# danielreardon/scintools

Hardware: NVIDIA H100
Metric: theta-theta eta-trials/sec on 4096x8192 dynspec (higher is better)
Workload: dtype f32

## Files before the change

profiles/probe_build_gather.py:

```python
import argparse
import ctypes
import json
import os
import subprocess
import sys

ROOT = os.path.dirname(os.path.dirname(os.path.abspath(__file__)))
sys.path.insert(0, ROOT)
import numpy as np
import torch

import bench as B
from scintools_b200 import _device as D, _lib, ththmod as thth


def load(path):
    lib = ctypes.CDLL(os.path.abspath(path))
    for name in ("sb_init", "sb_last_error", "sb_profile_enable", "sb_profile_collect",
                 "sb_eta_sweep", "sb_cs_f32", "sb_cs_bound_f32", "sb_release"):
        fn, ref = getattr(lib, name), getattr(_lib.lib, name)
        fn.restype, fn.argtypes = ref.restype, ref.argtypes
    if lib.sb_init(torch.cuda.current_device()) != 0:
        raise RuntimeError(lib.sb_last_error().decode())
    return lib


def check(lib, rc):
    if rc != 0:
        raise RuntimeError("error %d: %s" % (rc, lib.sb_last_error().decode()))


def stats(v):
    v = np.asarray(v, float)
    return {"min": float(v.min()), "median": float(np.median(v)), "max": float(v.max())}


def main():
    ap = argparse.ArgumentParser()
    ap.add_argument("libs", nargs="+", help="name=path, the first one is the reference")
    ap.add_argument("--rounds", type=int, default=10)
    ap.add_argument("--steps", type=int, default=20)
    ap.add_argument("--warmup", type=int, default=3)
    ap.add_argument("--out", default=None)
    a = ap.parse_args()
    card = subprocess.run(["nvidia-smi", "--query-gpu=name,power.limit,clocks.max.sm",
                           "--format=csv,noheader"], capture_output=True, text=True).stdout.strip()
    print("card:", card)
    D.device()
    libs = [(s.split("=", 1)[0], load(s.split("=", 1)[1])) for s in a.libs]

    dyn, freq, t = B.make_dynspec()
    fd = np.asarray(thth.fft_axis(t, "mHz", B.NPAD))
    tau = np.asarray(thth.fft_axis(freq, "us", B.NPAD))
    edges = np.linspace(-B.EDGE_LIM, B.EDGE_LIM, B.NEDGE)
    rng = np.random.default_rng(11)
    lim_nu = B.EDGE_LIM * (1.0 - 1.0 / (B.NEDGE - 1))
    edges_nu = np.sort(rng.uniform(-lim_nu, lim_nu, B.NEDGE))
    d_dyn = D.upload(dyn)
    ntau, nfd = (B.NPAD + 1) * B.NF, (B.NPAD + 1) * B.NT
    pitch = nfd // 2 + 16
    d_cs = D.empty((ntau, pitch, 2), torch.float32)
    keep = thth.needed_fd_columns(fd, edges) or 0
    d_bound = D.empty((1,), torch.float32)
    cs = thth.DeviceCS(d_cs, nfd=nfd, ncols_valid=keep or None, bound=d_bound)
    stream = D.stream_ptr()

    def buffers(etas):
        n = len(etas)
        return dict(n=n, etas=D.upload(np.ascontiguousarray(etas)),
                    eigs=D.empty((n,), torch.float64), stat=D.empty((n,), torch.int32),
                    nred=D.empty((n,), torch.int32), iters=D.empty((n,), torch.int32))

    def sweep(lib, geom, buf):
        check(lib, lib.sb_eta_sweep(geom.ref, buf["etas"].data_ptr(), buf["n"], thth.DEFAULT_TOL, 0,
                                    buf["eigs"].data_ptr(), buf["stat"].data_ptr(),
                                    buf["nred"].data_ptr(), buf["iters"].data_ptr(), stream))

    def spectrum(lib):
        check(lib, lib.sb_cs_f32(d_dyn.data_ptr(), B.NF, B.NT, B.NPAD, 0.0, 0, 1, pitch, keep,
                                 d_cs.data_ptr(), stream))
        check(lib, lib.sb_cs_bound_f32(d_dyn.data_ptr(), B.NF, B.NT, B.NPAD, 0.0,
                                       d_bound.data_ptr(), stream))

    def timed(lib, step, steps):
        lib.sb_profile_enable(1)
        e0, e1 = torch.cuda.Event(enable_timing=True), torch.cuda.Event(enable_timing=True)
        torch.cuda.synchronize()
        e0.record()
        for _ in range(steps):
            step()
        e1.record()
        torch.cuda.synchronize()
        ms = np.zeros(16)
        cnt = np.zeros(16, dtype=np.int32)
        check(lib, lib.sb_profile_collect(ms.ctypes.data, cnt.ctypes.data, 16))
        lib.sb_profile_enable(0)
        kern = {n_: ms[i] / steps for i, n_ in enumerate(B.PROF_NAMES) if cnt[i]}
        return e0.elapsed_time(e1) / steps, kern

    def ab(label, geom, etas, with_cs, rounds, steps):
        buf = buffers(etas)
        res = {name: {"step_ms": [], "kernel_ms": {}} for name, _ in libs}
        outs = {}
        for name, lib in libs:
            def step(lib=lib):
                if with_cs:
                    spectrum(lib)
                sweep(lib, geom, buf)
            for _ in range(a.warmup):
                step()
            torch.cuda.synchronize()
            outs[name] = {k: buf[k].cpu().numpy().copy() for k in ("eigs", "stat", "nred", "iters")}
            res[name]["step"] = step
        for _ in range(rounds):
            for name, lib in libs:
                ms, kern = timed(lib, res[name]["step"], steps)
                res[name]["step_ms"].append(ms)
                for k, v in kern.items():
                    res[name]["kernel_ms"].setdefault(k, []).append(v)
        ref = outs[libs[0][0]]
        out = {}
        for name, _ in libs:
            o = outs[name]
            same = all(np.array_equal(o[k], ref[k], equal_nan=(k == "eigs")) for k in o)
            out[name] = {"step_ms": stats(res[name]["step_ms"]),
                         "kernel_ms": {k: stats(v) for k, v in res[name]["kernel_ms"].items()},
                         "bit_equal_to_" + libs[0][0]: bool(same)}
            print(label, name, json.dumps(out[name]))
        return out

    geom = thth._Geom(cs, tau, fd, edges, True)
    geom_nu = thth._Geom(cs, tau, fd, edges_nu, True)
    report = {"card": card, "rounds": a.rounds, "steps": a.steps}
    report["bench_step_1024_uniform"] = ab("bench_step_1024_uniform", geom, B.eta_grid(B.NETA), True,
                                           a.rounds, a.steps)
    spectrum(libs[0][1])
    torch.cuda.synchronize()
    short = max(3, a.rounds // 2)
    report["sweep_16_uniform"] = ab("sweep_16_uniform", geom, B.eta_grid(16), False, short, a.steps)
    report["sweep_1024_nonuniform"] = ab("sweep_1024_nonuniform", geom_nu, B.eta_grid(B.NETA), False,
                                         short, max(2, a.steps // 4))
    report["sweep_16_nonuniform"] = ab("sweep_16_nonuniform", geom_nu, B.eta_grid(16), False, short,
                                       a.steps)
    for _, lib in libs:
        lib.sb_release()
    line = json.dumps(report)
    print(line)
    if a.out:
        os.makedirs(os.path.dirname(os.path.abspath(a.out)), exist_ok=True)
        with open(a.out, "w") as fh:
            fh.write(line + "\n")


if __name__ == "__main__":
    main()
```

scintools_b200/csrc/eig_half.cu:

```cuda
#ifndef SB_HOST_EMU
#include <cuda_fp16.h>
#endif
#include <float.h>
#include <math.h>
#include <stdlib.h>

#include "lanczos.cuh"
#include "tma.cuh"

namespace sb {

enum { EB_ST_INDEX_ERROR = 1, EB_ST_ZERO_START = 2, EB_ST_TOO_SMALL = 4,
       EB_ST_NOT_CONVERGED = 8 };

constexpr int EB_THREADS = 256;
constexpr int EB_NW = EB_THREADS / 32;
constexpr int EB_NST = 2;
#ifdef SB_EB_SLOTS
constexpr int EB_SLOTS = SB_EB_SLOTS;
#else
constexpr int EB_SLOTS = 48;
#endif

__device__ __forceinline__ void ffma2(float2& acc, const float2 a, const float b) {
    acc.x = fmaf(a.x, b, acc.x);
    acc.y = fmaf(a.y, b, acc.y);
}

__device__ __forceinline__ float2 unpack_f16x2(const unsigned p) {
    __half2 h;
    *reinterpret_cast<unsigned*>(&h) = p;
    return __half22float2(h);
}

__device__ __forceinline__ unsigned pack_h2(const float lo, const float hi) {
#ifdef SB_HOST_EMU
    const __half2 h = __floats2half2_rn(lo, hi);
    return (unsigned)h.x | ((unsigned)h.y << 16);
#else
    unsigned r;
    asm("cvt.rn.f16x2.f32 %0, %1, %2;" : "=r"(r) : "f"(hi), "f"(lo));
    return r;
#endif
}

constexpr int EB_TC_NST = 5;
#define EB_OWN5(a, b, c, d, e, cnt) \
    ((unsigned)(a) | (unsigned)(b) << 5 | (unsigned)(c) << 10 | (unsigned)(d) << 15 | \
     (unsigned)(e) << 20 | (unsigned)(cnt) << 25)
__device__ __forceinline__ unsigned eb_own_pack(const int warp) {
    if (warp >= EB_NW) return 0u;
    return EB_OWN5(warp, 15 - warp, 16 + warp, 31 - warp, 0, 4);
}

#ifdef SB_HOST_EMU
inline void ldsm_x4(unsigned (&r)[4], smem_addr a) {
    unsigned long long all[32];
    emu::warp_gather((unsigned long long)(uintptr_t)a, all);
    const int lane = (int)(threadIdx.x & 31), g = lane >> 2, t = lane & 3;
    for (int i = 0; i < 4; ++i)
        std::memcpy(&r[i], (const unsigned char*)(uintptr_t)all[8 * i + g] + 4 * t, 4);
}
inline void ldsm_x4_t(unsigned (&r)[4], smem_addr a) {
    unsigned long long all[32];
    emu::warp_gather((unsigned long long)(uintptr_t)a, all);
    const int lane = (int)(threadIdx.x & 31), g = lane >> 2, t = lane & 3;
    for (int i = 0; i < 4; ++i) {
        unsigned short lo, hi;
        std::memcpy(&lo, (const unsigned char*)(uintptr_t)all[8 * i + 2 * t] + 2 * g, 2);
        std::memcpy(&hi, (const unsigned char*)(uintptr_t)all[8 * i + 2 * t + 1] + 2 * g, 2);
        r[i] = (unsigned)lo | ((unsigned)hi << 16);
    }
}
inline void mma16816(float (&d)[4], const unsigned (&a)[4], const unsigned b0, const unsigned b1) {
    unsigned long long A01[32], A23[32], Bq[32];
    emu::warp_gather((unsigned long long)a[0] | ((unsigned long long)a[1] << 32), A01);
    emu::warp_gather((unsigned long long)a[2] | ((unsigned long long)a[3] << 32), A23);
    emu::warp_gather((unsigned long long)b0 | ((unsigned long long)b1 << 32), Bq);
    const int lane = (int)(threadIdx.x & 31), g = lane >> 2, t = lane & 3;
    auto half_of = [](unsigned w, int hi) { return emu_h2f((unsigned short)(hi ? w >> 16 : w & 0xffffu)); };
    auto Aat = [&](int row, int k) {
        const int ln = (row & 7) * 4 + ((k & 7) >> 1);
        const unsigned long long w = (k < 8) ? A01[ln] : A23[ln];
        return half_of((unsigned)(row < 8 ? w : w >> 32), k & 1);
    };
    auto Bat = [&](int k, int n) {
        const unsigned long long w = Bq[n * 4 + ((k & 7) >> 1)];
        return half_of((unsigned)(k < 8 ? w : w >> 32), k & 1);
    };
    for (int q = 0; q < 4; ++q) {
        const int row = g + 8 * (q >> 1), col = 2 * t + (q & 1);
        float acc = d[q];
        for (int k = 0; k < 16; ++k) acc += Aat(row, k) * Bat(k, col);
        d[q] = acc;
    }
}
#else
__device__ __forceinline__ void ldsm_x4(unsigned (&r)[4], const smem_addr a) {
    asm volatile("ldmatrix.sync.aligned.m8n8.x4.shared.b16 {%0, %1, %2, %3}, [%4];"
                 : "=r"(r[0]), "=r"(r[1]), "=r"(r[2]), "=r"(r[3]) : "r"(a) : "memory");
}
__device__ __forceinline__ void ldsm_x4_t(unsigned (&r)[4], const smem_addr a) {
    asm volatile("ldmatrix.sync.aligned.m8n8.x4.trans.shared.b16 {%0, %1, %2, %3}, [%4];"
                 : "=r"(r[0]), "=r"(r[1]), "=r"(r[2]), "=r"(r[3]) : "r"(a) : "memory");
}
__device__ __forceinline__ void mma16816(float (&d)[4], const unsigned (&a)[4], const unsigned b0,
                                         const unsigned b1) {
    asm("mma.sync.aligned.m16n8k16.row.col.f32.f16.f16.f32 {%0, %1, %2, %3}, {%4, %5, %6, %7}, "
        "{%8, %9}, {%0, %1, %2, %3};"
        : "+f"(d[0]), "+f"(d[1]), "+f"(d[2]), "+f"(d[3])
        : "r"(a[0]), "r"(a[1]), "r"(a[2]), "r"(a[3]), "r"(b0), "r"(b1));
}
#endif

__host__ __device__ constexpr size_t eig_half_slice() {
    return (size_t)EB_TC_NST * 1024 + 4096;
}
__host__ __device__ inline size_t eig_half_smem(int ld) {
    return sizeof(LanczosShared) + 4 * (size_t)ld * sizeof(float2) +
           (size_t)EB_NW * eig_half_slice() + (size_t)EB_NW * EB_NST * 8 + 16 +
           4 * (size_t)(ld / 2) * 8;
}

__global__ void __launch_bounds__(EB_THREADS + 32, 2)
thth_eig_half_kernel(const float2* __restrict__ Mbase, const unsigned* __restrict__ Mbbase,
                     int ld, const int* __restrict__ nred, int eta0,
                     double* __restrict__ eigs, int* __restrict__ status,
                     int* __restrict__ iters, double tol, double etol, double etol_h, double rtol_r,
                     int max_iter, float2* __restrict__ gbasis) {
    extern __shared__ __align__(128) unsigned char smem_raw[];
    LanczosShared& S = *reinterpret_cast<LanczosShared*>(smem_raw);
    float2* v = reinterpret_cast<float2*>(smem_raw + sizeof(LanczosShared));
    float2* vp = v + ld;
    float2* w = vp + ld;
    float2* u = w + ld;
    unsigned char* ring = reinterpret_cast<unsigned char*>(u + ld);
    float2* part = reinterpret_cast<float2*>(ring);
    constexpr int WSL = (int)eig_half_slice();
    static_assert(WSL >= EB_NST * 4096, "the fp32 pass needs two 4 KB stages per warp");
    unsigned long long* mbar = reinterpret_cast<unsigned long long*>(ring + (size_t)EB_NW * WSL);
    uint2* P = reinterpret_cast<uint2*>(reinterpret_cast<unsigned char*>(mbar) +
                                        (size_t)EB_NW * EB_NST * 8 + 16);
    const int tid = threadIdx.x, lane = tid & 31;
    const int warp = __shfl_sync(0xffffffffu, tid >> 5, 0);
    constexpr int CHKW = EB_NW;
    const bool worker = warp < EB_NW;
    const int tidw = worker ? tid : (1 << 24);
    const int e = blockIdx.x;
    const int n = nred[eta0 + e];
    const float2* M = Mbase + (size_t)e * ld * ld;
    const unsigned* Mb = Mbbase + (size_t)e * ld * ld;
    float2* basis = gbasis + (size_t)e * EB_SLOTS * ld;
    const double qnan = __longlong_as_double(0x7ff8000000000000LL);

    if (status[eta0 + e] & EB_ST_INDEX_ERROR) {
        if (tid == 0) { eigs[eta0 + e] = qnan; iters[eta0 + e] = 0; }
        return;
    }
    if (n < 3) {
        if (tid == 0) {
            eigs[eta0 + e] = qnan; iters[eta0 + e] = 0;
            status[eta0 + e] |= EB_ST_TOO_SMALL;
        }
        return;
    }
    for (int i = tidw; i < EB_NW * WSL / 16; i += EB_THREADS)
        reinterpret_cast<float4*>(ring)[i] = make_float4(0.f, 0.f, 0.f, 0.f);
    if (tid == 0) {
        for (int i = 0; i < EB_NW * EB_NST; ++i) mbar_init(mbar + i, 1);
        fence_mbarrier_init();
    }
    fence_proxy_async();
    __syncthreads();
    const int ncol4 = (n + 1) >> 1;
    unsigned char* mystage = ring + (size_t)warp * WSL;
    unsigned long long* mybar = mbar + EB_NST * warp;
    unsigned phbits = 0;

    auto matvec_t = [&](int check_m, double et) {
        const int ldh = ld >> 1;
        for (int c = tidw; c < ld; c += EB_THREADS) w[c] = make_float2(0.f, 0.f);
        for (int i = tidw; i < ldh; i += EB_THREADS) {
            const float4 x = *reinterpret_cast<const float4*>(v + 2 * i);
            const unsigned xr = pack_h2(x.x, x.z), xi = pack_h2(x.y, x.w);
            const float2 hr = unpack_f16x2(xr), hi = unpack_f16x2(xi);
            const unsigned lr = pack_h2((x.x - hr.x) * 2048.f, (x.z - hr.y) * 2048.f);
            const unsigned li = pack_h2((x.y - hi.x) * 2048.f, (x.w - hi.y) * 2048.f);
            const int q = (((i >> 3) << 2) + (i & 3)) * 2 + ((i >> 2) & 1);
            P[q] = make_uint2(xr, xi ^ 0x80008000u);
            P[ldh + q] = make_uint2(xi, xr);
            P[2 * ldh + q] = make_uint2(lr, li ^ 0x80008000u);
            P[3 * ldh + q] = make_uint2(li, lr);
        }
        unsigned char* wring = ring + (size_t)warp * WSL;
        float4* mypart = reinterpret_cast<float4*>(wring + EB_TC_NST * 1024);
        if (worker) {
#pragma unroll
            for (int i = 0; i < 8; ++i) mypart[lane + 32 * i] = make_float4(0.f, 0.f, 0.f, 0.f);
        }
        __syncthreads();
        const int g = lane >> 2, t = lane & 3;
        const int NI = (n + 14) >> 4;
        const int NH = (n + 15) >> 4;
        const int NGL = ld >> 3;
        const unsigned own = eb_own_pack(warp);
        const int cnt = (int)(own >> 25);
        const smem_addr sbase = smem_addr_of(wring);
        smem_addr cdst = sbase + lane * 16;
        const unsigned char* gsrc = reinterpret_cast<const unsigned char*>(Mb) + lane * 16;
        const int mi = lane >> 3;
        const int arow = (lane & 7) + 8 * (mi & 1), trow = (lane & 7) + 8 * (mi >> 1);
        smem_addr aoff = sbase + arow * 32 + ((((mi >> 1) & 1) ^ ((arow >> 2) & 1)) << 4);
        smem_addr toff = sbase + trow * 32 + (((mi & 1) ^ ((trow >> 2) & 1)) << 4);
#ifndef SB_HOST_EMU
        asm volatile("" : "+r"(cdst), "+r"(aoff), "+r"(toff), "+l"(gsrc));
#endif
        constexpr unsigned RING_BYTES = EB_TC_NST * 1024;
        int pj = -1, prem = 0;
        unsigned pa = 0u, pst = 0u;
        unsigned cst = 0u;
        bool pend = false;
        auto fetch_next = [&]() {
            if (prem == 0 && !pend) {
                for (;;) {
                    if (++pj >= cnt) { pend = true; break; }
                    const int I = (int)((own >> (5 * pj)) & 31u);
                    if (I < NI) {
                        prem = NH - I;
                        pa = (unsigned)(I * NGL + 2 * I) << 9;
                        break;
                    }
                }
            }
            if (!pend) {
                cp_async16_s(cdst + pst, gsrc + pa);
                cp_async16_s(cdst + pst + 512u, gsrc + pa + 512u);
                pa += 1024u;
                --prem;
            }
            pst += 1024u;
            if (pst == RING_BYTES) pst = 0u;
            cp_async_commit();
        };
        for (int k = 0; k < EB_TC_NST - 1; ++k) fetch_next();
        if (check_m > 0 && warp == CHKW) lanczos_check(S, check_m, tol, et);
        const float lo_scale = 1.f / 2048.f;
        const bool bact = g < 4;
        const uint4* Pg = reinterpret_cast<const uint4*>(P + (g & 3) * ldh) + t;
        for (int j = 0; j < cnt; ++j) {
            const int I = (int)((own >> (5 * j)) & 31u);
            if (I >= NI) continue;
            const uint4* pb = Pg + 4 * I;
            unsigned tb0 = 0u, tb1 = 0u;
            if (bact) { const uint4 e4 = *pb; tb0 = e4.x; tb1 = e4.z; }
            float acc[4] = {0.f, 0.f, 0.f, 0.f};
            float4* pc = mypart + 8 * I + g;
            for (int h = I; h < NH; ++h) {
                uint4 bq = make_uint4(0u, 0u, 0u, 0u);
                if (bact) bq = *pb;
                float4 q = make_float4(0.f, 0.f, 0.f, 0.f);
                if (t == 0) q = *pc;
                cp_async_wait<EB_TC_NST - 2>();
                __syncwarp();
                unsigned a0[4], t0[4], a1[4], t1[4];
                ldsm_x4(a0, aoff + cst);
                ldsm_x4_t(t0, toff + cst);
                ldsm_x4(a1, aoff + cst + 512u);
                ldsm_x4_t(t1, toff + cst + 512u);
                fetch_next();
                float c0[4] = {0.f, 0.f, 0.f, 0.f}, c1[4] = {0.f, 0.f, 0.f, 0.f};
                mma16816(acc, a0, bq.x, bq.y);
                mma16816(c0, t0, tb0, tb1);
                mma16816(acc, a1, bq.z, bq.w);
                mma16816(c1, t1, tb0, tb1);
                cst += 1024u;
                if (cst == RING_BYTES) cst = 0u;
                const float yr0 = c0[0] + c0[3], yi0 = c0[1] - c0[2];
                const float yr1 = c1[0] + c1[3], yi1 = c1[1] - c1[2];
                const float lr0 = __shfl_xor_sync(0xffffffffu, yr0, 1), li0 = __shfl_xor_sync(0xffffffffu, yi0, 1);
                const float lr1 = __shfl_xor_sync(0xffffffffu, yr1, 1), li1 = __shfl_xor_sync(0xffffffffu, yi1, 1);
                if (t == 0) {
                    q.x += fmaf(lr0, lo_scale, yr0);
                    q.y += fmaf(li0, lo_scale, yi0);
                    q.z += fmaf(lr1, lo_scale, yr1);
                    q.w += fmaf(li1, lo_scale, yi1);
                    *pc = q;
                }
                pb += 4;
                pc += 8;
            }
            const float l0 = __shfl_xor_sync(0xffffffffu, acc[0], 1);
            const float l1 = __shfl_xor_sync(0xffffffffu, acc[1], 1);
            const float l2 = __shfl_xor_sync(0xffffffffu, acc[2], 1);
            const float l3 = __shfl_xor_sync(0xffffffffu, acc[3], 1);
            if (t == 0) {
                w[16 * I + g] = make_float2(fmaf(l0, lo_scale, acc[0]), fmaf(l1, lo_scale, acc[1]));
                w[16 * I + g + 8] = make_float2(fmaf(l2, lo_scale, acc[2]), fmaf(l3, lo_scale, acc[3]));
            }
        }
        cp_async_wait<0>();
        __syncthreads();
        for (int c = tidw; c < ld; c += EB_THREADS) {
            float sx = 0.f, sy = 0.f;
            if (c < 16 * NH) {
                const int slot = (((c >> 4) << 3) + (c & 7)) * 2 + ((c >> 3) & 1);
#pragma unroll
                for (int kk = 0; kk < EB_NW; ++kk) {
                    const float2 q = reinterpret_cast<const float2*>(ring + (size_t)kk * WSL + EB_TC_NST * 1024)[slot];
                    sx += q.x;
                    sy += q.y;
                }
            }
            u[c] = make_float2(sx, sy);
        }
        __syncthreads();
    };

    auto matvec_f = [&]() {
        for (int c = tidw; c < ld; c += EB_THREADS) w[c] = make_float2(0.f, 0.f);
        __syncthreads();
        float4 yc[8];
#pragma unroll
        for (int j = 0; j < 8; ++j) yc[j] = make_float4(0.f, 0.f, 0.f, 0.f);
        const int K = (worker && n - 2 >= warp) ? (n - 2 - warp) / EB_NW + 1 : 0;
        auto issue = [&](int k) {
            const int a2 = warp + EB_NW * k;
            const int st = k % EB_NST;
            const int c_lo = (a2 + 1) & ~1;
            const unsigned bytes = (unsigned)(2 * ncol4 - c_lo) * 8u;
            mbar_expect_tx(mybar + st, bytes);
            bulk_g2s(mystage + st * 4096 + c_lo * 8, M + (size_t)a2 * ld + c_lo, bytes, mybar + st);
        };
        if (lane == 0)
            for (int k = 0; k < EB_NST && k < K; ++k) issue(k);
        for (int k = 0; k < K; ++k) {
            const int a = warp + EB_NW * k;
            const int first4 = (a + 1) >> 1;
            const float2 xa = v[a];
            const int st = k % EB_NST;
            while (!mbar_try_wait(mybar + st, (phbits >> st) & 1u)) {}
            phbits ^= 1u << st;
            const float4* sg = reinterpret_cast<const float4*>(mystage + st * 4096);
            float rx = 0.f, ry = 0.f;
            const int jskip = first4 >> 5;
#pragma unroll
            for (int j = 0; j < 8; ++j) {
                if (j < jskip) continue;
                const int c4 = lane + 32 * j;
                float4 q = make_float4(0.f, 0.f, 0.f, 0.f);
                if (c4 >= first4 && c4 < ncol4) q = sg[c4];
                const float4 x = (2 * c4 < ld) ? *reinterpret_cast<const float4*>(v + 2 * c4)
                                               : make_float4(0.f, 0.f, 0.f, 0.f);
                rx = fmaf(q.x, x.x, rx); rx = fmaf(-q.y, x.y, rx);
                rx = fmaf(q.z, x.z, rx); rx = fmaf(-q.w, x.w, rx);
                ry = fmaf(q.x, x.y, ry); ry = fmaf(q.y, x.x, ry);
                ry = fmaf(q.z, x.w, ry); ry = fmaf(q.w, x.z, ry);
                yc[j].x = fmaf(q.x, xa.x, yc[j].x); yc[j].x = fmaf(q.y, xa.y, yc[j].x);
                yc[j].y = fmaf(q.x, xa.y, yc[j].y); yc[j].y = fmaf(-q.y, xa.x, yc[j].y);
                yc[j].z = fmaf(q.z, xa.x, yc[j].z); yc[j].z = fmaf(q.w, xa.y, yc[j].z);
                yc[j].w = fmaf(q.z, xa.y, yc[j].w); yc[j].w = fmaf(-q.w, xa.x, yc[j].w);
            }
            __syncwarp();
            if (lane == 0 && k + EB_NST < K) issue(k + EB_NST);
            rx = warp_sum(rx);
            ry = warp_sum(ry);
            if (lane == 0) w[a] = make_float2(rx, ry);
        }
        __syncthreads();
        if (worker) {
#pragma unroll
            for (int j = 0; j < 8; ++j)
                *reinterpret_cast<float4*>(part + warp * 512 + 2 * (lane + 32 * j)) = yc[j];
        }
        __syncthreads();
        for (int c = tidw; c < 512; c += EB_THREADS) {
            float sx = 0.f, sy = 0.f;
#pragma unroll
            for (int kk = 0; kk < EB_NW; ++kk) { sx += part[kk * 512 + c].x; sy += part[kk * 512 + c].y; }
            if (c < ld) u[c] = make_float2(sx, sy);
        }
        __syncthreads();
        for (int i = tidw; i < EB_NW * WSL / 16; i += EB_THREADS)
            reinterpret_cast<float4*>(ring)[i] = make_float4(0.f, 0.f, 0.f, 0.f);
        fence_proxy_async();
        __syncthreads();
    };

    int m = 0;
    int mv = 0;
    auto lanczos_init = [&]() {
        if (tid == 0) {
            S.done = 0; S.lo = 0.0; S.theta = 0.0; S.res = 0.0;
            S.next_check = 1; S.m_last = 0; S.beta2[0] = 0.0;
        }
        __syncthreads();
    };
    auto step_scalars = [&](int it, float beta_prev, double& alpha, double& beta) {
        double apart = 0.0;
        for (int c = tidw; c < n; c += EB_THREADS) {
            float2 x = w[c];
            x.x += u[c].x;
            x.y += u[c].y;
            w[c] = x;
            apart += (double)(v[c].x * x.x + v[c].y * x.y);
        }
        apart = warp_sum(apart);
        if (lane == 0) S.red[0][warp] = apart;
        __syncthreads();
        alpha = 0.0;
        for (int k = 0; k < EB_NW; ++k) alpha += S.red[0][k];
        const float af = (float)alpha;
        double bpart = 0.0;
        for (int c = tidw; c < n; c += EB_THREADS) {
            float2 x = w[c];
            x.x -= af * v[c].x + beta_prev * vp[c].x;
            x.y -= af * v[c].y + beta_prev * vp[c].y;
            w[c] = x;
            bpart += (double)x.x * x.x + (double)x.y * x.y;
        }
        bpart = warp_sum(bpart);
        if (lane == 0) S.red[1][warp] = bpart;
        __syncthreads();
        double b2 = 0.0;
        for (int k = 0; k < EB_NW; ++k) b2 += S.red[1][k];
        beta = sqrt(b2);
        if (tid == 0) { S.alpha[it] = alpha; S.beta[it + 1] = beta; S.beta2[it + 1] = b2; }
        __syncthreads();
    };
    auto rotate = [&](double beta) {
        const float ib = (float)(1.0 / beta);
        for (int c = tidw; c < n; c += EB_THREADS) {
            const float2 x = w[c];
            vp[c] = v[c];
            v[c] = make_float2(x.x * ib, x.y * ib);
        }
        __syncthreads();
    };
    auto lanczos_b = [&](double et) -> bool {
        lanczos_init();
        float beta_prev = 0.f;
        m = 0;
        for (int it = 0; it < max_iter; ++it) {
            if (it >= EB_SLOTS) return false;
            for (int c = tidw; c < ld; c += EB_THREADS) basis[(size_t)it * ld + c] = v[c];
            const bool chk = it >= 1 && it >= S.next_check;
            matvec_t(chk ? it : 0, et);
            ++mv;
            double alpha, beta;
            step_scalars(it, beta_prev, alpha, beta);
            if (chk && S.done) { m = it; break; }
            m = it + 1;
            if (it + 1 == max_iter || !(beta > 0.0)) {
                if (warp == CHKW) lanczos_check(S, m, tol, et);
                __syncthreads();
                break;
            }
            if (!isfinite(alpha)) break;
            rotate(beta);
            beta_prev = (float)beta;
        }
        return true;
    };
    auto lanczos_f = [&](double et) {
        lanczos_init();
        float beta_prev = 0.f;
        m = 0;
        for (int it = 0; it < max_iter; ++it) {
            matvec_f();
            ++mv;
            double alpha, beta;
            step_scalars(it, beta_prev, alpha, beta);
            m = it + 1;
            const bool last = (it + 1 == max_iter);
            if (warp == 0 && (m >= S.next_check || last || !(beta > 0.0)))
                lanczos_check(S, m, tol, et);
            __syncthreads();
            if (S.done || !isfinite(alpha)) break;
            rotate(beta);
            beta_prev = (float)beta;
        }
    };

    auto start_vector = [&]() -> bool {
        const int h = n / 2;
        double part0 = 0.0;
        for (int c = tidw; c < ld; c += EB_THREADS) {
            float2 x = make_float2(0.f, 0.f);
            if (c < n && c > h) x = M[(size_t)h * ld + c];
            else if (c < h) { x = M[(size_t)c * ld + h]; x.y = -x.y; }
            v[c] = x;
            vp[c] = make_float2(0.f, 0.f);
            part0 += (double)x.x * x.x + (double)x.y * x.y;
        }
        part0 = warp_sum(part0);
        __syncthreads();
        if (lane == 0) S.red[0][warp] = part0;
        __syncthreads();
        double nrm2 = 0.0;
        for (int k = 0; k < EB_NW; ++k) nrm2 += S.red[0][k];
        if (!(nrm2 > 0.0) || !isfinite(nrm2)) return false;
        const float s = (float)(1.0 / sqrt(nrm2));
        for (int c = tidw; c < ld; c += EB_THREADS) { v[c].x *= s; v[c].y *= s; }
        __syncthreads();
        return true;
    };

    if (!start_vector()) {
        if (tid == 0) {
            eigs[eta0 + e] = qnan; iters[eta0 + e] = 0;
            status[eta0 + e] |= EB_ST_ZERO_START;
        }
        return;
    }
    const bool fits = lanczos_b(etol_h);
    bool plain = !fits || !S.done;
    if (!fits) {
        start_vector();
        lanczos_f(etol);
    } else if (S.done) {
        if (tid == 0) {
            const double theta = S.theta;
            double* s = S.piv;
            s[m - 1] = 1.0;
            if (m >= 2) s[m - 2] = (S.beta[m - 1] != 0.0) ? (theta - S.alpha[m - 1]) / S.beta[m - 1] : 0.0;
            for (int i = m - 2; i >= 1; --i) {
                const double t = (theta - S.alpha[i]) * s[i] - S.beta[i + 1] * s[i + 1];
                s[i - 1] = (S.beta[i] != 0.0) ? t / S.beta[i] : 0.0;
                if (fabs(s[i - 1]) > 1e150)
                    for (int k = i - 1; k < m; ++k) s[k] *= 1e-150;
            }
            double nn = 0.0;
            for (int i = 0; i < m; ++i) nn += s[i] * s[i];
            nn = 1.0 / sqrt(nn);
            for (int i = 0; i < m; ++i) s[i] *= nn;
        }
        __syncthreads();
        for (int c = tidw; c < ld; c += EB_THREADS) {
            float sx = 0.f, sy = 0.f;
            if (c < n) {
                for (int j = 0; j < m; ++j) {
                    const float2 q = basis[(size_t)j * ld + c];
                    const float sj = (float)S.piv[j];
                    sx = fmaf(sj, q.x, sx);
                    sy = fmaf(sj, q.y, sy);
                }
            }
            v[c] = make_float2(sx, sy);
            vp[c] = make_float2(0.f, 0.f);
        }
        __syncthreads();
        matvec_f();
        double num = 0.0, den = 0.0;
        for (int c = tidw; c < n; c += EB_THREADS) {
            const float2 y = v[c];
            float2 ay = w[c];
            ay.x += u[c].x;
            ay.y += u[c].y;
            w[c] = ay;
            num += (double)y.x * ay.x + (double)y.y * ay.y;
            den += (double)y.x * y.x + (double)y.y * y.y;
        }
        num = warp_sum(num);
        den = warp_sum(den);
        if (lane == 0) { S.red[0][warp] = num; S.red[1][warp] = den; }
        __syncthreads();
        double sn = 0.0, sd = 0.0;
        for (int k = 0; k < EB_NW; ++k) { sn += S.red[0][k]; sd += S.red[1][k]; }
        const double rho = (sd > 0.0) ? sn / sd : 0.0;
        __syncthreads();
        double rpart = 0.0;
        for (int c = tidw; c < n; c += EB_THREADS) {
            const double rx = (double)w[c].x - rho * v[c].x, ry = (double)w[c].y - rho * v[c].y;
            rpart += rx * rx + ry * ry;
        }
        rpart = warp_sum(rpart);
        if (lane == 0) S.red[0][warp] = rpart;
        __syncthreads();
        double r2 = 0.0;
        for (int k = 0; k < EB_NW; ++k) r2 += S.red[0][k];
        const bool accept = (sd > 0.0) && isfinite(rho) &&
                            (r2 <= rtol_r * rtol_r * rho * rho * sd);
        __syncthreads();
        if (accept) {
            if (tid == 0) { eigs[eta0 + e] = fabs(rho); iters[eta0 + e] = mv + 1; }
            return;
        }
        const float s = (sd > 0.0) ? (float)(1.0 / sqrt(sd)) : 0.f;
        for (int c = tidw; c < ld; c += EB_THREADS) { v[c].x *= s; v[c].y *= s; }
        __syncthreads();
        if (!(sd > 0.0)) start_vector();
        lanczos_f(etol);
        ++mv;
        plain = true;
    } else {
    }
    if (plain && tid == 0) {
        eigs[eta0 + e] = fabs(S.theta);
        iters[eta0 + e] = mv;
        if (!S.done) status[eta0 + e] |= EB_ST_NOT_CONVERGED;
    }
}

#ifndef SB_HOST_EMU
int eig_half_launch(const float2* d_M, const unsigned* d_Mb, int ld, const int* d_nred, int e0,
                    int nb, double* d_eigs, int* d_status, int* d_iters, double tol, double etol,
                    int max_iter, cudaStream_t st) {
    float2* d_basis = (float2*)workspace(7, (size_t)nb * EB_SLOTS * ld * sizeof(float2));
    if (!d_basis) return SB_ERR_NOMEM;
    double rtol_r = 1e-3;
    if (const char* ev = getenv("SB_EIG_RTOL_R")) rtol_r = atof(ev);
    double etol_h = 1e-6;
    if (const char* ev = getenv("SB_EIG_ETOL_B")) etol_h = atof(ev);
    const size_t smem = eig_half_smem(ld);
    SB_CUDA(cudaFuncSetAttribute(thth_eig_half_kernel, cudaFuncAttributeMaxDynamicSharedMemorySize,
                                 (int)smem));
    thth_eig_half_kernel<<<nb, EB_THREADS + 32, smem, st>>>(d_M, d_Mb, ld, d_nred, e0, d_eigs,
                                                            d_status, d_iters, tol, etol, etol_h,
                                                            rtol_r, max_iter, d_basis);
    SB_LAUNCH_CHECK();
    return SB_OK;
}
#endif

}
```

scintools_b200/csrc/tma.cuh:

```cuda
#pragma once

#ifdef SB_HOST_EMU
namespace sb {
inline void mbar_init(unsigned long long* bar, int) { *bar = 0; }
inline void mbar_expect_tx(unsigned long long* bar, unsigned bytes) {
    *bar += (unsigned long long)bytes << 8;
}
inline void bulk_g2s(void* dst, const void* src, unsigned bytes, unsigned long long* bar) {
    std::memcpy(dst, src, bytes);
    *bar -= (unsigned long long)bytes << 8;
    if ((*bar >> 8) == 0) *bar ^= 1ull;
}
inline bool mbar_try_wait(unsigned long long* bar, unsigned parity) {
    if ((unsigned)(*bar & 1ull) != parity) return true;
    emu::yield();
    return false;
}
inline void fence_mbarrier_init() {}
inline void fence_proxy_async() {}
inline void cp_async16(void* dst, const void* src) { std::memcpy(dst, src, 16); }
typedef unsigned char* smem_addr;
inline smem_addr smem_addr_of(void* p) { return (smem_addr)p; }
inline void cp_async16_s(smem_addr dst, const void* src) { std::memcpy(dst, src, 16); }
inline void cp_async_commit() {}
template <int N> inline void cp_async_wait() {}
}
#else

namespace sb {

__device__ __forceinline__ unsigned smem_u32(const void* p) {
    return (unsigned)__cvta_generic_to_shared(p);
}
__device__ __forceinline__ void mbar_init(unsigned long long* bar, int count) {
    asm volatile("mbarrier.init.shared::cta.b64 [%0], %1;" ::"r"(smem_u32(bar)), "r"(count));
}
__device__ __forceinline__ void mbar_expect_tx(unsigned long long* bar, unsigned bytes) {
    asm volatile("mbarrier.arrive.expect_tx.shared::cta.b64 _, [%0], %1;"
                 ::"r"(smem_u32(bar)), "r"(bytes) : "memory");
}
__device__ __forceinline__ void bulk_g2s(void* dst, const void* src, unsigned bytes,
                                         unsigned long long* bar) {
    asm volatile(
        "cp.async.bulk.shared::cluster.global.mbarrier::complete_tx::bytes [%0], [%1], %2, [%3];"
        ::"r"(smem_u32(dst)), "l"(src), "r"(bytes), "r"(smem_u32(bar)) : "memory");
}
__device__ __forceinline__ bool mbar_try_wait(unsigned long long* bar, unsigned parity) {
    unsigned ok;
    asm volatile(
        "{\n\t.reg .pred p;\n\t"
        "mbarrier.try_wait.parity.shared::cta.b64 p, [%1], %2;\n\t"
        "selp.u32 %0, 1, 0, p;\n\t}"
        : "=r"(ok) : "r"(smem_u32(bar)), "r"(parity) : "memory");
    return ok != 0;
}

__device__ __forceinline__ void fence_mbarrier_init() {
    asm volatile("fence.mbarrier_init.release.cluster;" ::: "memory");
}
__device__ __forceinline__ void cp_async16(void* dst, const void* src) {
    asm volatile("cp.async.cg.shared.global [%0], [%1], 16;" ::"r"(smem_u32(dst)), "l"(src) : "memory");
}
typedef unsigned smem_addr;
__device__ __forceinline__ smem_addr smem_addr_of(void* p) { return smem_u32(p); }
__device__ __forceinline__ void cp_async16_s(smem_addr dst, const void* src) {
    asm volatile("cp.async.cg.shared.global [%0], [%1], 16;" ::"r"(dst), "l"(src) : "memory");
}
__device__ __forceinline__ void cp_async_commit() {
    asm volatile("cp.async.commit_group;" ::: "memory");
}
template <int N> __device__ __forceinline__ void cp_async_wait() {
    asm volatile("cp.async.wait_group %0;" ::"n"(N) : "memory");
}
__device__ __forceinline__ void fence_proxy_async() {
    asm volatile("fence.proxy.async.shared::cta;" ::: "memory");
}

}
#endif
```

Baseline: 130,900.

## Pin a per-warp share of the half-precision matrix in L2 with eviction hints

Adds L2 cache-policy hints to the Lanczos eigen kernel's loads. Each worker warp marks the first part of its FP16 matrix stream as evict_last and the rest, plus the FP32 bulk loads, as evict_first. The goal is to keep a fixed slice (about 55% of L2 split across resident blocks) hot across Lanczos iterations instead of re-streaming it from HBM. Blocks reset the priority to normal on exit, and the hinted variant is used only when the matrix does not already fit in that budget. The risks are extra instructions per load and unpin traffic, and L2 thrashing if the share estimate is wrong.

```diff
diff --git a/profiles/probe_build_gather.py b/profiles/probe_build_gather.py
--- a/profiles/probe_build_gather.py
+++ b/profiles/probe_build_gather.py
@@ -33,6 +33,19 @@
 def stats(v):
     v = np.asarray(v, float)
     return {"min": float(v.min()), "median": float(np.median(v)), "max": float(v.max())}
+
+
+def eig_bytes(nred, iters):
+    total = 0
+    for n, it in zip(np.asarray(nred, np.int64), np.asarray(iters, np.int64)):
+        if n < 3 or it < 1:
+            continue
+        ni, nh = (n + 14) // 16, (n + 15) // 16
+        fp16 = 1024 * sum(nh - i for i in range(ni))
+        c_end = 2 * ((n + 1) // 2)
+        fp32 = 8 * sum(c_end - ((a + 1) & ~1) for a in range(n - 1))
+        total += (it - 1) * fp16 + fp32
+    return int(total)
 
 
 def main():
@@ -123,8 +136,11 @@
         for name, _ in libs:
             o = outs[name]
             same = all(np.array_equal(o[k], ref[k], equal_nan=(k == "eigs")) for k in o)
+            nbytes = eig_bytes(o["nred"], o["iters"])
+            eig_ms = np.median(res[name]["kernel_ms"]["thth_eig"])
             out[name] = {"step_ms": stats(res[name]["step_ms"]),
                          "kernel_ms": {k: stats(v) for k, v in res[name]["kernel_ms"].items()},
+                         "eig_bytes": nbytes, "eig_gbs": nbytes / (eig_ms * 1e6),
                          "bit_equal_to_" + libs[0][0]: bool(same)}
             print(label, name, json.dumps(out[name]))
         return out
diff --git a/scintools_b200/csrc/eig_half.cu b/scintools_b200/csrc/eig_half.cu
--- a/scintools_b200/csrc/eig_half.cu
+++ b/scintools_b200/csrc/eig_half.cu
@@ -48,10 +48,12 @@
 #define EB_OWN5(a, b, c, d, e, cnt) \
     ((unsigned)(a) | (unsigned)(b) << 5 | (unsigned)(c) << 10 | (unsigned)(d) << 15 | \
      (unsigned)(e) << 20 | (unsigned)(cnt) << 25)
-__device__ __forceinline__ unsigned eb_own_pack(const int warp) {
+__host__ __device__ __forceinline__ unsigned eb_own_pack(const int warp) {
     if (warp >= EB_NW) return 0u;
     return EB_OWN5(warp, 15 - warp, 16 + warp, 31 - warp, 0, 4);
 }
+
+constexpr double EB_PIN_FRAC = 0.55;
 
 #ifdef SB_HOST_EMU
 inline void ldsm_x4(unsigned (&r)[4], smem_addr a) {
@@ -122,12 +124,13 @@
            4 * (size_t)(ld / 2) * 8;
 }
 
+template <bool HINT = true>
 __global__ void __launch_bounds__(EB_THREADS + 32, 2)
 thth_eig_half_kernel(const float2* __restrict__ Mbase, const unsigned* __restrict__ Mbbase,
                      int ld, const int* __restrict__ nred, int eta0,
                      double* __restrict__ eigs, int* __restrict__ status,
                      int* __restrict__ iters, double tol, double etol, double etol_h, double rtol_r,
-                     int max_iter, float2* __restrict__ gbasis) {
+                     int max_iter, float2* __restrict__ gbasis, int pin_units = 0) {
     extern __shared__ __align__(128) unsigned char smem_raw[];
     LanczosShared& S = *reinterpret_cast<LanczosShared*>(smem_raw);
     float2* v = reinterpret_cast<float2*>(smem_raw + sizeof(LanczosShared));
@@ -220,6 +223,7 @@
         unsigned pa = 0u, pst = 0u;
         unsigned cst = 0u;
         bool pend = false;
+        int pleft = pin_units;
         auto fetch_next = [&]() {
             if (prem == 0 && !pend) {
                 for (;;) {
@@ -233,10 +237,19 @@
                 }
             }
             if (!pend) {
-                cp_async16_s(cdst + pst, gsrc + pa);
-                cp_async16_s(cdst + pst + 512u, gsrc + pa + 512u);
+                if (!HINT) {
+                    cp_async16_s(cdst + pst, gsrc + pa);
+                    cp_async16_s(cdst + pst + 512u, gsrc + pa + 512u);
+                } else if (pleft > 0) {
+                    cp_async16_s_hint(cdst + pst, gsrc + pa, l2_policy_evict_last());
+                    cp_async16_s_hint(cdst + pst + 512u, gsrc + pa + 512u, l2_policy_evict_last());
+                } else {
+                    cp_async16_s_hint(cdst + pst, gsrc + pa, l2_policy_evict_first());
+                    cp_async16_s_hint(cdst + pst + 512u, gsrc + pa + 512u, l2_policy_evict_first());
+                }
                 pa += 1024u;
                 --prem;
+                --pleft;
             }
             pst += 1024u;
             if (pst == RING_BYTES) pst = 0u;
@@ -329,7 +342,11 @@
             const int c_lo = (a2 + 1) & ~1;
             const unsigned bytes = (unsigned)(2 * ncol4 - c_lo) * 8u;
             mbar_expect_tx(mybar + st, bytes);
-            bulk_g2s(mystage + st * 4096 + c_lo * 8, M + (size_t)a2 * ld + c_lo, bytes, mybar + st);
+            if (!HINT)
+                bulk_g2s(mystage + st * 4096 + c_lo * 8, M + (size_t)a2 * ld + c_lo, bytes, mybar + st);
+            else
+                bulk_g2s_hint(mystage + st * 4096 + c_lo * 8, M + (size_t)a2 * ld + c_lo, bytes,
+                              mybar + st, l2_policy_evict_first());
         };
         if (lane == 0)
             for (int k = 0; k < EB_NST && k < K; ++k) issue(k);
@@ -505,6 +522,22 @@
         return true;
     };
 
+    auto unpin = [&]() {
+        if (!HINT || !worker || pin_units <= 0) return;
+        const int NI = (n + 14) >> 4, NH = (n + 15) >> 4, NGL = ld >> 3;
+        const unsigned own = eb_own_pack(warp);
+        const unsigned char* mb = reinterpret_cast<const unsigned char*>(Mb);
+        int left = pin_units;
+        for (int j = 0; j < (int)(own >> 25) && left > 0; ++j) {
+            const int I = (int)((own >> (5 * j)) & 31u);
+            if (I >= NI) continue;
+            const int units = left < NH - I ? left : NH - I;
+            const unsigned char* row = mb + ((size_t)(I * NGL + 2 * I) << 9);
+            for (int l = lane; l < 8 * units; l += 32) l2_evict_normal_128(row + 128 * l);
+            left -= units;
+        }
+    };
+
     if (!start_vector()) {
         if (tid == 0) {
             eigs[eta0 + e] = qnan; iters[eta0 + e] = 0;
@@ -583,6 +616,7 @@
         __syncthreads();
         if (accept) {
             if (tid == 0) { eigs[eta0 + e] = fabs(rho); iters[eta0 + e] = mv + 1; }
+            unpin();
             return;
         }
         const float s = (sd > 0.0) ? (float)(1.0 / sqrt(sd)) : 0.f;
@@ -599,9 +633,18 @@
         iters[eta0 + e] = mv;
         if (!S.done) status[eta0 + e] |= EB_ST_NOT_CONVERGED;
     }
+    unpin();
 }
 
 #ifndef SB_HOST_EMU
+constexpr int EB_MAX_DEVICES = 64;
+struct EigHalfDevice {
+    bool ready = false;
+    int nsm = 0, l2 = 0;
+    int occ[512 / 32 + 1] = {};
+};
+static EigHalfDevice eig_half_device[EB_MAX_DEVICES];
+
 int eig_half_launch(const float2* d_M, const unsigned* d_Mb, int ld, const int* d_nred, int e0,
                     int nb, double* d_eigs, int* d_status, int* d_iters, double tol, double etol,
                     int max_iter, cudaStream_t st) {
@@ -612,11 +655,44 @@
     double etol_h = 1e-6;
     if (const char* ev = getenv("SB_EIG_ETOL_B")) etol_h = atof(ev);
     const size_t smem = eig_half_smem(ld);
-    SB_CUDA(cudaFuncSetAttribute(thth_eig_half_kernel, cudaFuncAttributeMaxDynamicSharedMemorySize,
-                                 (int)smem));
-    thth_eig_half_kernel<<<nb, EB_THREADS + 32, smem, st>>>(d_M, d_Mb, ld, d_nred, e0, d_eigs,
-                                                            d_status, d_iters, tol, etol, etol_h,
-                                                            rtol_r, max_iter, d_basis);
+    int dev = 0;
+    SB_CUDA(cudaGetDevice(&dev));
+    if (dev < 0 || dev >= EB_MAX_DEVICES) return SB_ERR_ARG;
+    EigHalfDevice& D = eig_half_device[dev];
+    if (!D.ready) {
+        for (auto k : {thth_eig_half_kernel<true>, thth_eig_half_kernel<false>})
+            SB_CUDA(cudaFuncSetAttribute(k, cudaFuncAttributeMaxDynamicSharedMemorySize,
+                                         (int)eig_half_smem(512)));
+        SB_CUDA(cudaDeviceGetAttribute(&D.nsm, cudaDevAttrMultiProcessorCount, dev));
+        SB_CUDA(cudaDeviceGetAttribute(&D.l2, cudaDevAttrL2CacheSize, dev));
+        D.ready = true;
+    }
+    int& occ = D.occ[ld / 32];
+    if (occ == 0)
+        SB_CUDA(cudaOccupancyMaxActiveBlocksPerMultiprocessor(&occ, thth_eig_half_kernel<true>,
+                                                              EB_THREADS + 32, smem));
+    const int nsm = D.nsm, l2 = D.l2;
+    const long long resident = std::max(1LL, std::min((long long)nb, (long long)occ * nsm));
+    const int nh = ld >> 4;
+    int longest = 0;
+    for (int w = 0; w < EB_NW; ++w) {
+        const unsigned own = eb_own_pack(w);
+        int units = 0;
+        for (int j = 0; j < (int)(own >> 25); ++j) {
+            const int I = (int)((own >> (5 * j)) & 31u);
+            if (I < nh) units += nh - I;
+        }
+        longest = std::max(longest, units);
+    }
+    const long long share = (long long)(EB_PIN_FRAC * l2 / ((double)resident * EB_NW * 1024.0));
+    if (share < longest)
+        thth_eig_half_kernel<true><<<nb, EB_THREADS + 32, smem, st>>>(
+            d_M, d_Mb, ld, d_nred, e0, d_eigs, d_status, d_iters, tol, etol, etol_h, rtol_r, max_iter,
+            d_basis, (int)share);
+    else
+        thth_eig_half_kernel<false><<<nb, EB_THREADS + 32, smem, st>>>(
+            d_M, d_Mb, ld, d_nred, e0, d_eigs, d_status, d_iters, tol, etol, etol_h, rtol_r, max_iter,
+            d_basis);
     SB_LAUNCH_CHECK();
     return SB_OK;
 }
diff --git a/scintools_b200/csrc/tma.cuh b/scintools_b200/csrc/tma.cuh
--- a/scintools_b200/csrc/tma.cuh
+++ b/scintools_b200/csrc/tma.cuh
@@ -24,6 +24,21 @@
 inline void cp_async16_s(smem_addr dst, const void* src) { std::memcpy(dst, src, 16); }
 inline void cp_async_commit() {}
 template <int N> inline void cp_async_wait() {}
+typedef unsigned long long l2_policy;
+inline void (*emu_l2_hook)(const void* p, l2_policy pol, int kind) = nullptr;
+constexpr l2_policy EMU_POLICY_EVICT_FIRST = 1ull, EMU_POLICY_EVICT_LAST = 2ull;
+inline l2_policy l2_policy_evict_first() { return EMU_POLICY_EVICT_FIRST; }
+inline l2_policy l2_policy_evict_last() { return EMU_POLICY_EVICT_LAST; }
+inline void cp_async16_s_hint(smem_addr dst, const void* src, l2_policy pol) {
+    if (emu_l2_hook) emu_l2_hook(src, pol, 0);
+    std::memcpy(dst, src, 16);
+}
+inline void bulk_g2s_hint(void* dst, const void* src, unsigned bytes, unsigned long long* bar, l2_policy) {
+    bulk_g2s(dst, src, bytes, bar);
+}
+inline void l2_evict_normal_128(const void* p) {
+    if (emu_l2_hook) emu_l2_hook(p, 0ull, 1);
+}
 }
 #else
 
@@ -72,6 +87,31 @@
 template <int N> __device__ __forceinline__ void cp_async_wait() {
     asm volatile("cp.async.wait_group %0;" ::"n"(N) : "memory");
 }
+typedef unsigned long long l2_policy;
+__device__ __forceinline__ l2_policy l2_policy_evict_first() {
+    l2_policy p;
+    asm volatile("createpolicy.fractional.L2::evict_first.b64 %0, 1.0;" : "=l"(p));
+    return p;
+}
+__device__ __forceinline__ l2_policy l2_policy_evict_last() {
+    l2_policy p;
+    asm volatile("createpolicy.fractional.L2::evict_last.b64 %0, 1.0;" : "=l"(p));
+    return p;
+}
+__device__ __forceinline__ void cp_async16_s_hint(smem_addr dst, const void* src, l2_policy pol) {
+    asm volatile("cp.async.cg.shared.global.L2::cache_hint [%0], [%1], 16, %2;"
+                 ::"r"(dst), "l"(src), "l"(pol) : "memory");
+}
+__device__ __forceinline__ void bulk_g2s_hint(void* dst, const void* src, unsigned bytes,
+                                              unsigned long long* bar, l2_policy pol) {
+    asm volatile(
+        "cp.async.bulk.shared::cluster.global.mbarrier::complete_tx::bytes.L2::cache_hint"
+        " [%0], [%1], %2, [%3], %4;"
+        ::"r"(smem_u32(dst)), "l"(src), "r"(bytes), "r"(smem_u32(bar)), "l"(pol) : "memory");
+}
+__device__ __forceinline__ void l2_evict_normal_128(const void* p) {
+    asm volatile("applypriority.global.L2::evict_normal [%0], 128;" ::"l"(p) : "memory");
+}
 __device__ __forceinline__ void fence_proxy_async() {
     asm volatile("fence.proxy.async.shared::cta;" ::: "memory");
 }
```

Measured after the change: 138,700 (median of 6 runs). 5.9% higher.
